# nk4517/gaussian-splatting-skysphere

Hardware: AMD Instinct MI355X
Metric: train iters/sec (fwd+bwd) + render Mpix/s @1080p, 1M Gaussians SH=3 (higher is better)
Workload: dtype f32; 1 GPU; C3: 1M Gaussians SH3 1920x1080, 16x16 tiles; gaussians=1000000, sh_degree=3, width=1920, height=1080, render_exp2=hardware v_exp_f32, parallelism=view-parallel dp1

## Files before the change

### gaussian-splatting-skysphere_amd/csrc/gs_api.hip

```cpp
#include <dlfcn.h>

#include <atomic>
#include <cstdlib>
#include <stdarg.h>
#include <stdio.h>
#include <string.h>

#include <mutex>
#include <string>
#include <vector>

#include "../../include/gsrast.h"
#include "gs_internal.h"

namespace gs {

static thread_local std::string t_err;
static thread_local bool t_failed = false;
static thread_local bool t_debug = false;

static void set_error(const char* fmt, ...) {
  if (t_failed) return;
  char buf[1024];
  va_list ap;
// ... 202 lines not shown
  }
  if (rgb) {
    rgb[3 * i] = b.z;
    rgb[3 * i + 1] = b.w;
    rgb[3 * i + 2] = d.x;
  }
  if (depth) depth[i] = d.y;
}

}

using namespace gs;

namespace gs {
static std::atomic<int> g_exact_exp{-1};
bool exact_exp() {
  int v = g_exact_exp.load(std::memory_order_relaxed);
  if (v < 0) {
    const char* e = getenv("GSRAST_EXACT_EXP");
    v = (e && e[0] && e[0] != '0') ? 1 : 0;
    g_exact_exp.store(v, std::memory_order_relaxed);
  }
  return v != 0;
}
}

namespace gs {
static std::atomic<uint32_t> g_spin_limit{LB_SPIN_LIMIT};
uint32_t scan_spin_limit() { return g_spin_limit.load(std::memory_order_relaxed); }
static std::atomic<int> g_tile_sort_packed{1};
static std::atomic<long long> g_tile_sort_packed_n{0};
bool tile_sort_packed() { return g_tile_sort_packed.load(std::memory_order_relaxed) != 0; }
void tile_sort_packed_note() { g_tile_sort_packed_n.fetch_add(1, std::memory_order_relaxed); }

static thread_local RowWait t_row_waits[GS_MAX_ROW_WAITS];
static thread_local int t_row_wait_count = 0;
int take_row_waits(RowWait* out, int max) {
  const int n = t_row_wait_count < max ? t_row_wait_count : max;
  for (int k = 0; k < n; k++) out[k] = t_row_waits[k];
  t_row_wait_count = 0;
  return n;
}
bool stream_wait(hipStream_t st, hipEvent_t ev) {
  const hipError_t e = hipStreamWaitEvent(st, ev, 0);
  if (e != hipSuccess) set_error("row wait: hipStreamWaitEvent failed: %s", hipGetErrorString(e));
  return e == hipSuccess;
}
uint32_t next_scan_epoch() {
  static std::atomic<uint32_t> e{0};
  return (e.fetch_add(1, std::memory_order_relaxed) % ((1u << 30) - 1u)) + 1u;
}
}

extern "C" {

int gs_abi_version(void) { return GSRAST_ABI_VERSION; }
const char* gs_last_error(void) { return t_err.c_str(); }

size_t gs_geom_buffer_bytes(int P) { return geom_layout((size_t)(P > 0 ? P : 1), nullptr, nullptr); }
size_t gs_binning_buffer_bytes(long long num_rendered, int W, int H) {
  if (size_query_refused(W, H)) return 0;
  int tiles = ((W + GS_TILE - 1) / GS_TILE) * ((H + GS_TILE - 1) / GS_TILE);
  return bin_layout((size_t)(num_rendered > 0 ? num_rendered : 1), tiles, nullptr, nullptr);
}
size_t gs_image_buffer_bytes(int W, int H) {
  if (size_query_refused(W, H)) return 0;
// ... 1213 lines not shown
  bwd_gaussians_adam(g, c, geo, a, (hipStream_t)stream);
  return t_failed ? 1 : 0;
}

int gs_mark_visible(int P, const float* means3D, const float* viewmatrix, const float* projmatrix, uint8_t* present,
                    void* stream) {
  clear_error(0);
  if (P < 0) return set_error("P must be >= 0"), 1;
  if (P > 0 && (!means3D || !viewmatrix || !present)) return set_error("missing pointer"), 1;
  mark_visible(P, means3D, viewmatrix, projmatrix, present, (hipStream_t)stream);
  return t_failed ? 1 : 0;
}

size_t gs_knn_scratch_bytes(int P) { return knn_scratch_bytes(P); }

int gs_knn_mean_dist2(int P, const float* points, float* out, void* scratch, void* stream) {
  clear_error(0);
  if (P < 0) return set_error("P must be >= 0"), 1;
  if (P == 0) return 0;
  if (!points || !out || !scratch) return set_error("missing pointer"), 1;
  knn_mean_dist2(P, points, out, (char*)scratch, (hipStream_t)stream);
  return t_failed ? 1 : 0;
}

unsigned gs_debug_set_scan_spin_limit(unsigned limit) {
  return gs::g_spin_limit.exchange(limit, std::memory_order_relaxed);
}

int gs_debug_set_tile_sort_packed(int on) {
  return gs::g_tile_sort_packed.exchange(on ? 1 : 0, std::memory_order_relaxed);
}
long long gs_debug_tile_sort_packed_count(void) { return gs::g_tile_sort_packed_n.load(std::memory_order_relaxed); }

int gs_debug_sh_rows_staged(int D, int M, const void* shs) { return gs::sh_rows_stageable(D, M, shs) ? 1 : 0; }

int gs_debug_launch_log(int enable) {
  const int prev = gs::launch_log_on();
  gs::g_launch_log.store(enable ? 1 : 0, std::memory_order_relaxed);
  return prev;
}

long long gs_debug_launched_kernels(char* buf, long long cap) {
  std::string out;
  {
    std::lock_guard<std::mutex> lk(gs::g_launch_mu);
    for (const void* k : gs::g_launched) {
      Dl_info info;
      if (dladdr(k, &info) && info.dli_sname && info.dli_saddr == k)
        out += info.dli_sname;
      else
        out += "?";
      out += '\n';
    }
  }
  if (buf && cap > (long long)out.size()) memcpy(buf, out.c_str(), out.size() + 1);
  return (long long)out.size();
}

int gs_set_exact_exp(int exact) {
  const int prev = exact_exp() ? 1 : 0;
  gs::g_exact_exp.store(exact ? 1 : 0, std::memory_order_relaxed);
  return prev;
}

size_t gs_ssim_partial_count(int planes, int H, int W) { return ssim_partial_count(planes, H, W); }

// ... 364 lines not shown
```

### gaussian-splatting-skysphere_amd/csrc/gs_backward.hip

```cpp
#include "gs_internal.h"

namespace gs {

#ifdef GS_TIMING
GS_TIMING_BUFFER(g_bwd_timing, gs_debug_bwd_timing)
#define GS_BWD_T0() const unsigned long long t_start = timing_stamp()
#define GS_BWD_TREC(tile, n_eff, walked, slots) timing_record(g_bwd_timing, t_start, tile, n_eff, walked, slots)
#else
#define GS_BWD_T0() (void)0
#define GS_BWD_TREC(tile, n_eff, walked, slots) (void)0
#endif

struct __attribute__((aligned(4))) Rec3 {
  float a, b, c;
};

__device__ __forceinline__ void load_rec(const float* p, float* v) {
  const Rec3* r = reinterpret_cast<const Rec3*>(p);
  const Rec3 a = r[0], b = r[1], c = r[2];
  v[0] = a.a, v[1] = a.b, v[2] = a.c, v[3] = b.a, v[4] = b.b, v[5] = b.c, v[6] = c.a, v[7] = c.b, v[8] = c.c;
}


struct BwdSlot {
// ... 18 lines not shown
  if constexpr (EXACT) inv = __builtin_fmaf(inv, __builtin_fmaf(-omA, inv, 1.0f), inv);
  const float Tn = q.T * inv;
  const float dch = ae * Tn;
  float Cd = __builtin_fmaf(bl, q.d2, __builtin_fmaf(xr.w, q.d1, xr.z * q.d0));
  if constexpr (AUX) Cd = __builtin_fmaf(br.w, q.gD, Cd);
  const float dLa = __builtin_fmaf(Tn, Cd, -(q.U * inv));
  const float qq = oGm * dLa;
  const float mx = dx - br.y, my = dy - br.z;
  const float qx = qq * mx, qy = qq * my;
  s[0] = __builtin_fmaf(dch, q.d0, s[0]);
  s[1] = __builtin_fmaf(dch, q.d1, s[1]);
  s[2] = __builtin_fmaf(dch, q.d2, s[2]);
  s[3] = s[3] + qx;
  s[4] = s[4] + qy;
  s[5] = __builtin_fmaf(qx, mx, s[5]);
  s[6] = __builtin_fmaf(qx, my, s[6]);
  s[7] = __builtin_fmaf(qy, my, s[7]);
  s[8] = s[8] + qq;
  if constexpr (AUX) s[9] = __builtin_fmaf(dch, q.gD, s[9]);
  if constexpr (ABS) {
    constexpr int A0 = AUX ? GRAD_REC + 1 : GRAD_REC;
    const float hx = __builtin_fmaf(co.x + co.x, dx, co.y * dy);
    const float hy = __builtin_fmaf(co.z + co.z, dy, co.y * dx);
    s[A0] = __builtin_fmaf(__builtin_fabsf(qq), __builtin_fabsf(hx), s[A0]);
    s[A0 + 1] = __builtin_fmaf(__builtin_fabsf(qq), __builtin_fabsf(hy), s[A0 + 1]);
  }
  q.T = Tn;
  q.U = __builtin_fmaf(Cd, dch, q.U);
  uint64_t m = __builtin_amdgcn_ballot_w64(c_walk) & __builtin_amdgcn_ballot_w64(c_alpha);
  if constexpr (EXACT) m &= __builtin_amdgcn_ballot_w64(c_pw);
  return m;
}

template <bool EXACT, bool AUX = false, bool ABS = false, class... Abs>
__global__ __launch_bounds__(64) void k_render_bwd_tw(CameraArgs c, const uint2* __restrict__ ranges,
                                                                    const uint32_t* __restrict__ point_list,
                                                                    const uint32_t* __restrict__ point_gid,
                                                                    const float4* __restrict__ splat,
                                                                    const float* __restrict__ final_T,
                                                                    const uint32_t* __restrict__ n_contrib,
                                                                    const uint32_t* __restrict__ tile_max,
                                                                    const uint32_t* __restrict__ tile_order,
                                                                    const float* __restrict__ dL_dpix,
                                                                    float* __restrict__ gradrec, BwdAux aux,
                                                                    Abs... abs) {
  static_assert(sizeof...(Abs) == (ABS ? 1 : 0), "ABS: one BwdAbs argument");
  __shared__ float4 s_xy[64];
  __shared__ float4 s_co[64];
  __shared__ float4 s_br[64];
  constexpr int AOFF = AUX ? 24 : 16;
  constexpr int ROW = ABS ? (AUX ? 36 : 24) : AOFF;
  constexpr int NS = GRAD_REC + (AUX ? 1 : 0) + (ABS ? 2 : 0);
  __shared__ __attribute__((aligned(16))) float s_acc[64][ROW];
  GS_BWD_T0();
  const uint32_t tile = __builtin_amdgcn_readfirstlane(tile_order ? tile_order[blockIdx.x] : blockIdx.x);
  if (tile == ~0u) return;
  const int tx = (int)(tile % (uint32_t)c.gx), ty = (int)(tile / (uint32_t)c.gx);
  const int lane = threadIdx.x;
  const uint2 range = ranges[tile];
  const uint32_t n = range.y - range.x;
  const uint4 qm = reinterpret_cast<const uint4*>(tile_max)[tile];
  const uint32_t qlast[4] = {min(qm.x, n), min(qm.y, n), min(qm.z, n), min(qm.w, n)};
  const uint32_t n_eff = max(max(qlast[0], qlast[1]), max(qlast[2], qlast[3]));
  if (n_eff == 0) {
    GS_BWD_TREC(tile, 0u, 0u, 0u);
    return;
  }
#ifdef GS_TIMING
  uint32_t t_walked = 0, t_slots = 0;
#endif

  const size_t HW = (size_t)c.W * c.H;
  const int qx0 = tx * GS_TILE + (lane & 7), qy0 = ty * GS_TILE + (lane >> 3);
  BwdSlot p[4];
#pragma unroll
  for (int k = 0; k < 4; k++) {
    const int px = qx0 + 8 * (k & 1), py = qy0 + 8 * (k >> 1);
    const bool in = px < c.W && py < c.H;
    const size_t pix = in ? (size_t)py * c.W + px : 0;
    const float Tf = in ? final_T[pix] : 0.0f;
    p[k].T = Tf;
    p[k].last = in ? n_contrib[pix] : 0u;
    p[k].d0 = in ? dL_dpix[pix] : 0.0f;
    p[k].d1 = in ? dL_dpix[HW + pix] : 0.0f;
    p[k].d2 = in ? dL_dpix[2 * HW + pix] : 0.0f;
    p[k].U = Tf * (c.bg[0] * p[k].d0 + c.bg[1] * p[k].d1 + c.bg[2] * p[k].d2);
    if constexpr (AUX) {
      const float gA = in && aux.d_alpha ? aux.d_alpha[pix] : 0.0f;
      p[k].U = p[k].U - Tf * gA;
      p[k].gD = in && aux.d_invdepth ? aux.d_invdepth[pix] : 0.0f;
    }
  }
  const float ddelx_dx = (float)(0.5 * c.W), ddely_dy = (float)(0.5 * c.H);
  const float pfx0 = (float)qx0, pfy0 = (float)qy0;
  using lds_float = __attribute__((address_space(3))) float;
  lds_float* const acc_lane = (lds_float*)(&s_acc[0][(lane >> 4) + 4 * ((lane >> 3) & 1)]);
  const bool hi8 = (lane & 8) != 0;

  const int32_t e0 = (int32_t)n_eff - 1 - lane;
  const uint32_t* const plist = point_list + range.x;
  auto pos = [&](int32_t e) { return (uint32_t)max(e, 0); };
  uint32_t slot_c = plist[pos(e0)];
  uint32_t G1 = point_gid[slot_c];
  float4 pa = splat[3 * G1], pb = splat[3 * G1 + 1], pd = splat[3 * G1 + 2];
  uint32_t S1 = plist[pos(e0 - 64)];
  G1 = point_gid[S1];
  uint32_t S2 = plist[pos(e0 - 128)];

  uint32_t rec_lanes = 0;
  auto store_records = [&]() {
    if ((uint32_t)lane < rec_lanes) {
      const float4* row = reinterpret_cast<const float4*>(&s_acc[lane][0]);
      const float4 a = row[0], b = row[1], d = row[2];
      Rec3* r = reinterpret_cast<Rec3*>(gradrec + (size_t)__float_as_uint(d.y) * GRAD_REC);
      r[0] = Rec3{a.x, a.y, a.z};
      r[1] = Rec3{a.w, b.x, b.y};
      r[2] = Rec3{b.z, b.w, d.x};
      if constexpr (AUX) aux.gradrec_aux[__float_as_uint(d.y)] = d.z;
      if constexpr (ABS) {
        const float4 ea = row[3];
        reinterpret_cast<float2*>((abs, ...).gradrec_abs)[__float_as_uint(d.y)] = make_float2(ea.x, ea.y);
      }
    }
  };
  for (uint32_t base = 0; base < n_eff; base += 64) {
    const uint32_t cnt = min(64u, n_eff - base);
    const bool mine = (uint32_t)lane < cnt;
    const uint32_t slot = slot_c;
    const float ccx = pa.z, ccy = pa.w, ccz = pb.x, cop = pb.y;
    uint32_t qmask = 0;
    if (mine) {
      s_xy[lane] = make_float4(pa.x, pa.y, pb.z, pb.w);
      s_co[lane] = fall_coefs_m<EXACT>(pa.z, pa.w, pb.x, pb.y);
      const float x0 = (float)(tx * GS_TILE), y0 = (float)(ty * GS_TILE);
      s_br[lane] = make_float4(pd.x, pa.x - fminf(fmaxf(pa.x, x0), x0 + 15.0f),
// ... 79 lines not shown
        if constexpr (ABS) {
          const float4 b0 = *reinterpret_cast<const float4*>(&s_acc[lane][AOFF]);
          const float4 b1 = *reinterpret_cast<const float4*>(&s_acc[lane][AOFF + 4]);
          S[NS - 2] = (b0.x + b1.x) + (b0.y + b1.y);
          S[NS - 1] = (b0.z + b1.z) + (b0.w + b1.w);
        }
      } else {
#pragma unroll
        for (int t = 0; t < NS; t++) S[t] = 0.0f;
      }
      const float2 R = *reinterpret_cast<const float2*>(&s_br[lane].y);
      const double Rx = R.x, Ry = R.y, q0 = S[8];
      const float m1x = (float)__builtin_fma(Rx, q0, (double)S[3]), m1y = (float)__builtin_fma(Ry, q0, (double)S[4]);
      __builtin_amdgcn_sched_barrier(0);
      const float m2xx = (float)__builtin_fma(Rx, __builtin_fma(Rx, q0, 2.0 * (double)S[3]), (double)S[5]);
      __builtin_amdgcn_sched_barrier(0);
      const float m2xy = (float)__builtin_fma(Rx, __builtin_fma(Ry, q0, (double)S[4]),
                                              __builtin_fma(Ry, (double)S[3], (double)S[6]));
      __builtin_amdgcn_sched_barrier(0);
      const float m2yy = (float)__builtin_fma(Ry, __builtin_fma(Ry, q0, 2.0 * (double)S[4]), (double)S[7]);
      __builtin_amdgcn_sched_barrier(0);
      float4* row = reinterpret_cast<float4*>(&s_acc[lane][0]);
      row[0] = make_float4(S[0], S[1], S[2], -ddelx_dx * (ccx * m1x + ccy * m1y));
      row[1] = make_float4(-ddely_dy * (ccz * m1y + ccy * m1x), -0.5f * m2xx, -0.5f * m2xy, -0.5f * m2yy);
      float s9 = 0.0f;
      if constexpr (AUX) s9 = S[9];
      row[2] = make_float4(S[8] != 0.0f ? S[8] / cop : 0.0f, __uint_as_float(slot), s9, 0.0f);
      if constexpr (ABS) row[3] = make_float4(S[NS - 2], S[NS - 1], 0.0f, 0.0f);
    }
    rec_lanes = cnt;
    __builtin_amdgcn_wave_barrier();
  }
  store_records();
  GS_BWD_TREC(tile, n_eff, t_walked, t_slots);
}

constexpr int ORDER_THREADS = 256;
__global__ __launch_bounds__(ORDER_THREADS) void k_tile_order(const uint32_t* __restrict__ len_hist,
                                                              const uint32_t* __restrict__ tile_brank, uint32_t gx,
                                                              uint32_t gy, uint32_t* __restrict__ order,
                                                              const uint32_t* __restrict__ tile_max,
                                                              const uint2* __restrict__ ranges,
                                                              const uint32_t* __restrict__ point_list,
                                                              uint32_t* __restrict__ tile_cut,
                                                              uint32_t* __restrict__ cut_max) {
  __shared__ uint32_t s_base[ORDER_GROUPS][ORDER_BUCKETS];
  const uint32_t tid = threadIdx.x, t = blockIdx.x * ORDER_THREADS + tid, lane = tid & 63, wid = tid >> 6;
  const uint32_t tiles = gx * gy;
  uint32_t cut = 0;
  if (t < tiles) {
    const uint4 q = reinterpret_cast<const uint4*>(tile_max)[t];
    const uint2 r = ranges[t];
    const uint32_t n_eff = min(max(max(q.x, q.y), max(q.z, q.w)), r.y - r.x);
    cut = n_eff ? point_list[r.x + n_eff - 1] + 1u : 0u;
    tile_cut[t] = cut;
  }
  {
    const uint32_t wm = wave_max_u32(cut);
    if (lane == 0 && wm) atomicMax(cut_max, wm);
  }
  if (!order) return;
  const uint32_t br = t < tiles ? tile_brank[t] : 0u;
  static_assert(ORDER_BUCKETS == 64 && ORDER_GROUPS == 2 * (ORDER_THREADS / 64), "two groups per wave");
#pragma unroll
  for (int h = 0; h < 2; h++) {
    const uint32_t g = wid + h * (ORDER_THREADS / 64);
    const uint32_t v = len_hist[g * ORDER_BUCKETS + lane];
    s_base[g][lane] = wave_incl_scan(v) - v;
  }
  lds_barrier();
  if (t < tiles) {
    const uint32_t g = t % ORDER_GROUPS;
    order[ORDER_GROUPS * (s_base[g][br >> 22] + (br & 0x3FFFFFu)) + g] = t;
  }
}

void bwd_tile_order(const CameraArgs& c, const BinPtrs& bin, const ImgPtrs& img, hipStream_t st) {
  const uint32_t slots = (uint32_t)(c.gx * c.gy);
  GS_LAUNCH("tile_order", k_tile_order, dim3((slots + ORDER_THREADS - 1) / ORDER_THREADS), dim3(ORDER_THREADS), 0, st,
            img.len_hist, img.tile_brank, (uint32_t)c.gx, (uint32_t)c.gy, img.tile_order, img.tile_max, img.ranges,
            bin.point_list, img.tile_cut, img.cut_max);
}

void bwd_render(int P, const CameraArgs& c, const GeomPtrs& geo, const BinPtrs& bin, const ImgPtrs& img,
                const float* dL_dpix, float* gradrec, hipStream_t st, const BwdAux& aux, const BwdAbs& ab) {
  const int tiles = c.gx * c.gy;
  uint32_t* order = img.tile_order;
  const uint32_t slots = (uint32_t)tiles;
  bwd_tile_order(c, bin, img, st);
  auto launch = [&](const char* name, const char* name_aux, auto... abs) {
    with_flag(aux.on(), [&](auto AUX) {
      with_flag(exact_exp(), [&](auto EXACT) {
        constexpr bool E = decltype(EXACT)::value, A = decltype(AUX)::value;
        GS_LAUNCH(A ? name_aux : name, (k_render_bwd_tw<E, A, sizeof...(abs) != 0, decltype(abs)...>), dim3(slots),
                  dim3(64), 0, st, c, img.ranges, bin.point_list, bin.presort_gid, geo.splat, img.final_T,
                  img.n_contrib, img.tile_max, order, dL_dpix, gradrec, aux, abs...);
      });
    });
  };
  if (ab.on())
    launch("render_bwd_abs", "render_bwd_aux_abs", ab);
  else
    launch("render_bwd", "render_bwd_aux");
}

constexpr int SUMREC_WAVES = 4;
template <int CTRL, int ROW_MASK, int NC = GRAD_REC>
__device__ __forceinline__ void seg_scan_step(float* v, uint32_t own1) {
  const uint32_t o = (uint32_t)__builtin_amdgcn_update_dpp(0, (int)own1, CTRL, ROW_MASK, 0xF, false);
  const float f = o == own1 ? 1.0f : 0.0f;
#pragma unroll
  for (int c = 0; c < NC; c++) v[c] = __builtin_fmaf(dpp_f<CTRL, ROW_MASK>(v[c]), f, v[c]);
}

template <bool AUX = false, bool ABS = false, class... Abs>
__global__ __launch_bounds__(64 * SUMREC_WAVES) void k_sum_records(const uint32_t* __restrict__ counters,
                                                                   const uint32_t* __restrict__ offsets,
                                                                   const uint32_t* __restrict__ sorted_gid,
                                                                   const uint32_t* __restrict__ slot_tile,
                                                                   const uint32_t* __restrict__ tile_cut,
                                                                   const uint32_t* __restrict__ cut_max,
                                                                   const float* __restrict__ gradrec,
                                                                   float* __restrict__ gsum, uint32_t P,
                                                                   const float* __restrict__ gradrec_aux,
                                                                   float* __restrict__ gsum_aux, Abs... abs) {
  static_assert(sizeof...(Abs) == (ABS ? 1 : 0), "ABS: one BwdAbs argument");
  constexpr int A0 = AUX ? GRAD_REC + 1 : GRAD_REC;
  constexpr int NC = A0 + (ABS ? 2 : 0);
  [[maybe_unused]] const float2* gradrec_abs = nullptr;
// ... 1270 lines not shown
```

### gaussian-splatting-skysphere_amd/csrc/gs_forward.hip

```cpp
#include "gs_internal.h"

namespace gs {


template <int DEG>
__device__ __forceinline__ void sh_row_load(const float* __restrict__ sh, const float* __restrict__ rest, bool split,
                                            int M, float* s) {
  constexpr int K = (DEG + 1) * (DEG + 1);
  if (split) {
    const F3 d = *reinterpret_cast<const F3*>(sh);
    s[0] = d.a, s[1] = d.b, s[2] = d.c;
    const F3* r3 = reinterpret_cast<const F3*>(rest);
#pragma unroll
    for (int j = 0; j < K - 1; j++) {
      const F3 t = r3[j];
      s[3 + 3 * j] = t.a, s[4 + 3 * j] = t.b, s[5 + 3 * j] = t.c;
    }
  } else if (((M * 3) & 3) == 0) {
    const float4* s4 = reinterpret_cast<const float4*>(sh);
#pragma unroll
    for (int v = 0; v < (K * 3 + 3) / 4; v++) {
      float4 q = s4[v];
      if (4 * v + 0 < K * 3) s[4 * v + 0] = q.x;
      if (4 * v + 1 < K * 3) s[4 * v + 1] = q.y;
// ... 921 lines not shown
        m_cu &= ~m_stop;
        const bool cu = __builtin_amdgcn_inverse_ballot_w64(m_cu);
        px.C0 = cu ? px.C0 + rr * al[u] * px.T : px.C0;
        px.C1 = cu ? px.C1 + rg * al[u] * px.T : px.C1;
        px.C2 = cu ? px.C2 + rb * al[u] * px.T : px.C2;
        if constexpr (AUX) px.D = cu ? px.D + rd * al[u] * px.T : px.D;
        px.T = cu ? tT : px.T;
        px.last = cu ? __float_as_uint(bl.y) : px.last;
      } else {
        const float tT = __builtin_fmaf(-al[u], px.T, px.T);
        const uint64_t m_keep = __builtin_amdgcn_ballot_w64(tT >= 0.0001f);
        px.done |= m_cu & ~m_keep;
        m_cu &= m_keep;
        const bool cu = __builtin_amdgcn_inverse_ballot_w64(m_cu);
        const float wgt = cu ? al[u] * px.T : 0.0f;
        px.C0 = __builtin_fmaf(rr, wgt, px.C0);
        px.C1 = __builtin_fmaf(rg, wgt, px.C1);
        px.C2 = __builtin_fmaf(rb, wgt, px.C2);
        if constexpr (AUX) px.D = __builtin_fmaf(rd, wgt, px.D);
        px.T = cu ? tT : px.T;
        px.last = cu ? __float_as_uint(bl.y) : px.last;
      }
    }
    if (px.done == ~0ull) break;
  }
}

#ifdef GS_TIMING
GS_TIMING_BUFFER(g_fwd_timing, gs_debug_fwd_timing)
#endif

__device__ __forceinline__ void tile_finish(uint32_t tile, uint32_t grp, uint32_t wave_last,
                                            uint64_t* __restrict__ tile_done, uint32_t* __restrict__ len_hist,
                                            uint32_t* __restrict__ tile_brank) {
  const uint32_t cls = min((uint32_t)(4.0f * __log2f((float)wave_last + 1.0f)), 47u);
  const uint64_t mine = (1ull << (8 + cls)) + 1ull;
  const uint64_t old = atomicAdd((unsigned long long*)&tile_done[tile], (unsigned long long)mine);
  if ((old & 7ull) != 3ull) return;
  const uint32_t top = 63u - (uint32_t)__builtin_clzll((old + mine) >> 8);
  const uint32_t b = (uint32_t)ORDER_BUCKETS - 1u - top;
  tile_brank[tile] = b << 22 | atomicAdd(&len_hist[grp * ORDER_BUCKETS + b], 1u);
}

__device__ __forceinline__ void fwd_store(const CameraArgs& c, const QuadPix& q, bool inside, const FwdPix& px,
                                          float* __restrict__ out, float* __restrict__ final_T,
                                          uint32_t* __restrict__ n_contrib) {
  if (inside) {
    const size_t pix = (size_t)q.py * c.W + q.px, HW = (size_t)c.W * c.H;
    final_T[pix] = px.T;
    n_contrib[pix] = px.last;
    out[pix] = px.C0 + px.T * c.bg[0];
    out[HW + pix] = px.C1 + px.T * c.bg[1];
    out[2 * HW + pix] = px.C2 + px.T * c.bg[2];
  }
}
__device__ __forceinline__ void fwd_store_aux(const CameraArgs& c, const QuadPix& q, bool inside, const FwdPix& px,
                                              float* __restrict__ out_invdepth, float* __restrict__ out_alpha) {
  if (inside) {
    const size_t pix = (size_t)q.py * c.W + q.px;
    if (out_invdepth) out_invdepth[pix] = px.D;
    if (out_alpha) out_alpha[pix] = 1.0f - px.T;
  }
}

constexpr int FWDQ_NB = 64;
constexpr int FWDQ_NBS = FWDQ_NB + 1;
template <bool EXACT, bool AUX = false>
__global__ __launch_bounds__(64) void k_render_fwd_q(CameraArgs c, const uint2* __restrict__ ranges,
                                                     const uint32_t* __restrict__ point_list,
                                                     const uint32_t* __restrict__ point_gid,
                                                     const float4* __restrict__ splat, float* __restrict__ out,
                                                     ImgPtrs img, const uint32_t* __restrict__ err,
                                                     uint32_t* __restrict__ err_host, FwdAux aux) {
  __shared__ float4 s_ent[3 * FWDQ_NBS];
// ... 21 lines not shown
  FwdPix px;
  px.done = __builtin_amdgcn_ballot_w64(!inside);
  for (uint32_t base = 0; base < n; base += FWDQ_NB) {
    if (px.done == ~0ull) break;
    bool meets = false;
    if (lane < (uint32_t)FWDQ_NB && base + lane < n) {
      const uint32_t gid = point_gid[point_list[range.x + base + lane]];
      const float4 a = splat[3 * gid], bb = splat[3 * gid + 1], d = splat[3 * gid + 2];
      s_ent[lane] = make_float4(a.x, a.y, bb.z, bb.w);
      s_ent[FWDQ_NBS + lane] = fall_coefs_m<EXACT>(a.z, a.w, bb.x, bb.y);
      s_ent[2 * FWDQ_NBS + lane] =
          make_float4(d.x, __uint_as_float(base + lane + 1), AUX ? 1.0f / d.y : 0.0f, 0.0f);
      meets = d.z >= 0.0f && ellipse_meets_rect(a.x, a.y, a.z, a.w, bb.x, d.z, qx, qx + 7.0f, qy, qy + 7.0f);
    }
    const uint64_t m = __ballot(meets);
    if (meets)
      s_qlist[__builtin_amdgcn_mbcnt_hi((uint32_t)(m >> 32), __builtin_amdgcn_mbcnt_lo((uint32_t)m, 0u))] =
          16u * lane;
    const uint32_t qcnt = (uint32_t)__popcll(m);
    if (lane < 2 * FWD_ILP) s_qlist[qcnt + lane] = 16u * FWDQ_NB;
    __builtin_amdgcn_wave_barrier();
#ifdef GS_TIMING
    t_batches++;
    t_walked += qcnt;
#endif
    fwd_walk<EXACT, FWDQ_NBS, AUX>(ent, s_qlist, qcnt, (float)q.px, (float)q.py, px);
    __builtin_amdgcn_wave_barrier();
  }
  fwd_store(c, q, inside, px, out, img.final_T, img.n_contrib);
  if constexpr (AUX) fwd_store_aux(c, q, inside, px, aux.invdepth, aux.alpha);
  const uint32_t wmax = wave_max_u32(px.last);
  if (lane == 0) {
    img.tile_max[4 * tile + wid] = wmax;
    tile_finish(tile, tile % ORDER_GROUPS, wmax, img.tile_done, img.len_hist, img.tile_brank);
  }
#ifdef GS_TIMING
  timing_record(g_fwd_timing, t_start, tile, (uint32_t)wid | n << 2, t_batches, t_walked);
#endif
}

void fwd_render(const CameraArgs& c, const GeomPtrs& geo, const BinPtrs& bin, const ImgPtrs& img, float* out_color,
                hipStream_t st, uint32_t* err_host, const FwdAux& aux) {
  const int tiles = c.gx * c.gy;
  const int blocks = (int)xcd_span((uint32_t)tiles) * 32;
  with_flag(aux.invdepth || aux.alpha, [&](auto AUX) {
    with_flag(exact_exp(), [&](auto EXACT) {
      GS_LAUNCH(decltype(AUX)::value ? "render_fwd_aux" : "render_fwd",
                (k_render_fwd_q<decltype(EXACT)::value, decltype(AUX)::value>), dim3(blocks), dim3(64), 0, st, c,
                img.ranges, bin.point_list, bin.presort_gid, geo.splat, out_color, img, &geo.counters[CNT_ERR], err_host,
                aux);
    });
  });
}

__global__ __launch_bounds__(256) void k_mark_visible(int P, const float* __restrict__ means,
                                                      const float* __restrict__ view, uint8_t* __restrict__ present) {
  const int i = blockIdx.x * 256 + threadIdx.x;
  if (i >= P) return;
  const float3v pv = xf43(view, means[3 * i], means[3 * i + 1], means[3 * i + 2]);
  present[i] = !(pv.z <= 0.2f);
}

void mark_visible(int P, const float* means3D, const float* view, const float* proj, uint8_t* present,
                  hipStream_t st) {
  (void)proj;
  if (P <= 0) return;
  GS_LAUNCH("mark_visible", k_mark_visible, dim3((P + 255) / 256), dim3(256), 0, st, P, means3D, view, present);
// ... 4 lines not shown
```

### gaussian-splatting-skysphere_amd/csrc/gs_internal.h

```cpp
#pragma once
#include <stddef.h>
#include <stdint.h>

#include <cmath>
#include <type_traits>

#include "../../include/gsrast.h"
#include "gs_common.h"
#include "gs_sortscan.h"

namespace gs {

bool exact_exp();


constexpr int GRAD_REC = 9;

inline size_t align_up(size_t x) { return (x + 255) & ~(size_t)255; }

constexpr uint32_t DUP_SLOTS = 2048;
__host__ __device__ inline bool dup_balanced(uint32_t I, uint32_t P) {
  return (uint64_t)I <= (uint64_t)DUP_SLOTS * (uint64_t)P;
}

// ... 178 lines not shown
    out->vals_a = (uint32_t*)(base + o_va);
    out->keys_b = (uint32_t*)(base + o_kb);
    out->vals_b = (uint32_t*)(base + o_vb);
    out->offsets = (uint32_t*)(base + o_offs);
    out->rtiles_a = (uint32_t*)(base + o_rta);
    out->rtiles_b = (uint32_t*)(base + o_rtb);
    out->tiles_by_rank = (radix_passes(32) % 2 == 0) ? out->rtiles_b : out->rtiles_a;
    out->dup_first = (uint32_t*)(base + o_df);
    out->gsum = (float*)(base + o_gs);
    out->scan_partial = (uint32_t*)(base + o_sp);
    out->lb_status = (uint64_t*)(base + o_lb);
    out->sort_scratch = (uint32_t*)(base + o_ss);
    out->counters = (uint32_t*)(base + o_cnt);
    out->wg_tot = (WgTotals*)(base + o_wg);
    out->sorted_gid = (radix_passes(32) % 2 == 0) ? out->vals_a : out->vals_b;
  }
  return off;
}

struct BinPtrs {
  uint32_t *keys_a, *vals_a, *keys_b, *vals_b;
  uint32_t* presort_gid;
  uint32_t* sort_scratch;
  uint32_t* point_list;
  uint32_t* sorted_tile;
  uint32_t* slot_tile;
  uint32_t* count;
  uint32_t* pack_tab;
};

constexpr size_t PACK_SCRATCH_WORDS = (size_t)RADIX * RADIX;
bool tile_sort_packed();
void tile_sort_packed_note();



inline int tile_bits(int tiles) {
  int b = 1;
  while (b < 32 && ((uint64_t)1 << b) < (uint64_t)tiles) b++;
  return b;
}

inline size_t bin_layout(size_t I, int tiles, BinPtrs* out, char* base) {
  size_t off = 0;
  auto take = [&](size_t bytes) {
    size_t o = off;
    off += align_up(bytes);
    return o;
  };
  size_t In = I ? I : 1;
  size_t o_ka = take(In * 4), o_va = take(In * 4), o_kb = take(In * 4), o_vb = take(In * 4);
  size_t o_pg = take(In * 4), o_st = take(In * 4);
  size_t o_ss = take((sort_scratch_words(In) + PACK_SCRATCH_WORDS) * 4);
  size_t o_cn = take(64);
  size_t o_pt = take(PACK_TAB_WORDS * 4);
  if (out && base) {
    out->count = (uint32_t*)(base + o_cn);
    out->pack_tab = (uint32_t*)(base + o_pt);
    out->keys_a = (uint32_t*)(base + o_ka);
    out->vals_a = (uint32_t*)(base + o_va);
    out->keys_b = (uint32_t*)(base + o_kb);
    out->vals_b = (uint32_t*)(base + o_vb);
    out->presort_gid = (uint32_t*)(base + o_pg);
    out->slot_tile = (uint32_t*)(base + o_st);
    out->sort_scratch = (uint32_t*)(base + o_ss);
    bool in_b = radix_passes(tile_bits(tiles)) % 2 == 1;
    out->point_list = in_b ? out->vals_b : out->vals_a;
    out->sorted_tile = in_b ? out->keys_b : out->keys_a;
  }
  return off;
}

struct ImgPtrs {
  uint2* ranges;
  float* final_T;
  uint32_t* n_contrib;
  uint32_t* tile_max;
  uint32_t* tile_order;
  uint32_t* tile_cut;
  uint64_t* tile_done;
  uint32_t* len_hist;
  uint32_t* tile_brank;
  uint32_t* cut_max;
};

constexpr int ORDER_BUCKETS = 64;
inline uint32_t sched_words(uint32_t tiles);

constexpr int ORDER_GROUPS = 8;
inline uint32_t sched_words(uint32_t tiles) { return 2u * tiles + ORDER_GROUPS * ORDER_BUCKETS + 1u; }
__host__ __device__ inline uint32_t xcd_span(uint32_t tiles) { return (tiles + ORDER_GROUPS - 1) / ORDER_GROUPS; }
__host__ __device__ inline uint32_t xcd_tile(uint32_t g, uint32_t k, uint32_t gx, uint32_t gy) {
  const uint32_t t = ORDER_GROUPS * k + g;
  return t < gx * gy ? t : ~0u;
}

inline size_t img_layout(int W, int H, ImgPtrs* out, char* base) {
  size_t off = 0;
  auto take = [&](size_t bytes) {
    size_t o = off;
    off += align_up(bytes);
    return o;
  };
  size_t tiles = (size_t)((W + GS_TILE - 1) / GS_TILE) * ((H + GS_TILE - 1) / GS_TILE);
  size_t npix = (size_t)W * H;
  if (tiles == 0) tiles = 1;
  if (npix == 0) npix = 1;
  size_t o_r = take(tiles * 8), o_t = take(npix * 4), o_n = take(npix * 4), o_m = take(tiles * 16),
         o_o = take(tiles * 4), o_c = take(tiles * 4), o_d = take((size_t)sched_words((uint32_t)tiles) * 4),
         o_b = take(tiles * 4);
  if (out && base) {
    out->ranges = (uint2*)(base + o_r);
    out->final_T = (float*)(base + o_t);
    out->n_contrib = (uint32_t*)(base + o_n);
    out->tile_max = (uint32_t*)(base + o_m);
    out->tile_order = (uint32_t*)(base + o_o);
    out->tile_cut = (uint32_t*)(base + o_c);
    out->tile_done = (uint64_t*)(base + o_d);
    out->len_hist = (uint32_t*)(out->tile_done + tiles);
    out->cut_max = out->len_hist + ORDER_GROUPS * ORDER_BUCKETS;
    out->tile_brank = (uint32_t*)(base + o_b);
  }
  return off;
}

#ifdef GS_TIMING
constexpr int TIMING_MAX = 1 << 16;
#define GS_TIMING_BUFFER(buf, fn)                                                                   \
  __device__ unsigned long long buf[TIMING_MAX][5];                                                 \
  extern "C" int fn(unsigned long long* host_out, int n, int reset) {                               \
    if (n > TIMING_MAX) n = TIMING_MAX;                                                             \
    if (host_out && hipMemcpyFromSymbol(host_out, HIP_SYMBOL(buf), (size_t)n * 5 * 8) != hipSuccess) \
      return 1;                                                                                     \
    if (reset) {                                                                                    \
      void* p = nullptr;                                                                            \
      if (hipGetSymbolAddress(&p, HIP_SYMBOL(buf)) != hipSuccess) return 1;                          \
      if (hipMemset(p, 0, sizeof(buf)) != hipSuccess || hipDeviceSynchronize() != hipSuccess) return 1; \
    }                                                                                               \
    return 0;                                                                                       \
  }
__device__ __forceinline__ unsigned long long timing_stamp() {
  __builtin_amdgcn_sched_barrier(0);
  const unsigned long long t = __builtin_amdgcn_s_memrealtime();
  __builtin_amdgcn_s_waitcnt(0xC07F);
  __builtin_amdgcn_sched_barrier(0);
  return t;
}
__device__ __forceinline__ void timing_record(unsigned long long (*buf)[5], unsigned long long t0, uint32_t a,
                                              uint32_t b, uint32_t c, uint32_t d) {
  const unsigned long long t1 = timing_stamp();
  if (threadIdx.x == 0 && blockIdx.x < TIMING_MAX) {
    const uint32_t xcc = __builtin_amdgcn_s_getreg((31 << 11) | 20);
    const uint32_t hw = __builtin_amdgcn_s_getreg((31 << 11) | 4);
    unsigned long long* o = buf[blockIdx.x];
// ... 267 lines not shown
```

### gaussian-splatting-skysphere_amd/diff_gaussian_rasterization/_native.py

```python
from __future__ import annotations

import ctypes
import os

_PKG_ROOT = os.path.dirname(os.path.dirname(os.path.abspath(__file__)))
LIB_PATH = os.environ.get("GSRAST_LIB", os.path.join(_PKG_ROOT, "build", "libgsrast.so"))

_c_p = ctypes.c_void_p
_c_i = ctypes.c_int
_c_d = ctypes.c_double
_c_f = ctypes.c_float
_c_ll = ctypes.c_longlong
_c_sz = ctypes.c_size_t



class ViewGrad(ctypes.Structure):
    _fields_ = [("viewmatrix", ctypes.c_void_p), ("projmatrix", ctypes.c_void_p), ("campos", ctypes.c_void_p),
                ("tan_fovx", ctypes.c_float), ("tan_fovy", ctypes.c_float), ("image_width", ctypes.c_int),
                ("image_height", ctypes.c_int), ("geom_buffer", ctypes.c_void_p)]


SIGNATURES = {
    "gs_abi_version": (_c_i, []),
# ... 173 lines not shown
    "gs_sky_camera_scratch_bytes": (_c_sz, [_c_i, _c_i]),
    "gs_sky_compose_backward_camera": (_c_i, [_c_i, _c_i, _c_p, _c_f, _c_f, _c_i, _c_i, _c_p, _c_p, _c_p, _c_p, _c_p,
                                              _c_i, _c_p, _c_p, _c_i, _c_p, _c_p]),
    "gs_mark_visible": (_c_i, [_c_i, _c_p, _c_p, _c_p, _c_p, _c_p]),
    "gs_knn_scratch_bytes": (_c_sz, [_c_i]),
    "gs_knn_mean_dist2": (_c_i, [_c_i, _c_p, _c_p, _c_p, _c_p]),
    "gs_set_exact_exp": (_c_i, [_c_i]),
    "gs_debug_launch_log": (_c_i, [_c_i]),
    "gs_debug_launched_kernels": (_c_ll, [ctypes.c_char_p, _c_ll]),
    "gs_ssim_partial_count": (_c_sz, [_c_i, _c_i, _c_i]),
    "gs_ssim_forward": (_c_i, [_c_i, _c_i, _c_i, _c_p, _c_p, _c_p, _c_p, _c_p, _c_p, _c_p]),
    "gs_ssim_backward": (_c_i, [_c_i, _c_i, _c_i, _c_i, _c_p, _c_p, _c_p, _c_p, _c_p, _c_p, _c_p]),
    "gs_photometric_loss_forward": (_c_i, [_c_i, _c_i, _c_i, _c_p, _c_p, _c_p, _c_f, _c_p, _c_p, _c_p, _c_p]),
    "gs_photometric_loss_backward": (_c_i, [_c_i, _c_i, _c_i, _c_p, _c_p, _c_p, _c_p, _c_f, _c_p, _c_p, _c_p]),
    "gs_adam_step": (_c_i, [_c_i, _c_p, _c_p, _c_p, _c_p, _c_p, _c_p, _c_p, _c_p, _c_d, _c_d, _c_d, _c_i, _c_p]),
    "gs_adam_step_activated": (_c_i, [_c_i, _c_p, _c_p, _c_p, _c_i, _c_p, _c_p, _c_p, _c_p, _c_p, _c_p, _c_d, _c_d, _c_d,
                                      _c_i, _c_p]),
    "gs_activate_forward": (_c_i, [_c_i, _c_i] + [_c_p] * 9 + [_c_p]),
    "gs_activate_backward": (_c_i, [_c_i, _c_i] + [_c_p] * 12 + [_c_p]),
    "gs_densify_block_count": (_c_sz, [_c_i]),
    "gs_densify_classify": (_c_i, [_c_i, _c_p, _c_p, _c_p, _c_p, _c_d, _c_d, _c_d, _c_d, _c_i, _c_d, _c_i, _c_p, _c_p,
                                   _c_p, _c_p]),
    "gs_densify_split_stds": (_c_i, [_c_i, _c_i, _c_p, _c_p, _c_p, _c_p, _c_p, _c_p]),
    "gs_densify_emit": (_c_i, [_c_i, _c_i] + [_c_p] * 12),
    "gs_densify_stats": (_c_i, [_c_i, _c_p, _c_p, _c_i, _c_p, _c_p, _c_p, _c_p]),
    "gs_debug_export": (
        _c_i,
        [_c_i, _c_i, _c_i, _c_ll, _c_p, _c_p, _c_p, _c_p, _c_p, _c_p, _c_p, _c_p, _c_p, _c_p, _c_p, _c_p, _c_p],
    ),
    "gs_debug_export_slots": (_c_i, [_c_i, _c_i, _c_ll, _c_p, _c_p, _c_p, _c_p, _c_p]),
    "gs_debug_set_scan_spin_limit": (ctypes.c_uint, [ctypes.c_uint]),
    "gs_debug_set_tile_sort_packed": (_c_i, [_c_i]),
    "gs_debug_tile_sort_packed_count": (_c_ll, []),
    "gs_debug_sh_rows_staged": (_c_i, [_c_i, _c_i, _c_p]),
    "gs_profile_enable": (None, [_c_i]),
    "gs_profile_collect": (_c_i, []),
    "gs_profile_reset": (None, []),
    "gs_profile_stat": (_c_i, [_c_i, ctypes.c_char_p, _c_i, ctypes.POINTER(ctypes.c_double), ctypes.POINTER(_c_ll)]),
}

_lib = None


def load():
    global _lib
    if _lib is not None:
        return _lib
    if not os.path.exists(LIB_PATH):
        raise ImportError(
            f"libgsrast.so not found at {LIB_PATH}; build it with "
            f"`make -C {_PKG_ROOT}` (hipcc --offload-arch=gfx950). There is no CPU fallback."
        )
    lib = ctypes.CDLL(LIB_PATH, mode=ctypes.RTLD_GLOBAL)
    for name, (res, args) in SIGNATURES.items():
        fn = getattr(lib, name)
        fn.restype = res
        fn.argtypes = args
    _lib = lib
    return lib


def last_error() -> str:
    msg = load().gs_last_error()
    return msg.decode() if msg else "unknown error"


# ... 18 lines not shown
```

### include/gsrast.h

```cpp
#ifndef GSRAST_H
#define GSRAST_H

#include <stddef.h>
#include <stdint.h>

#ifdef __cplusplus
extern "C" {
#endif

#define GSRAST_ABI_VERSION 17

#define GSRAST_HAS_AUX 1

#define GSRAST_HAS_SKY 1

#define GSRAST_HAS_SKY_CAMERA 1

#define GSRAST_HAS_CAMERA_GRAD 1

#define GSRAST_HAS_AUX_DEFERRED 1

#define GSRAST_HAS_ANTIALIASING 1

#define GSRAST_HAS_CONTRIB 1
// ... 341 lines not shown
                        const float* opacity_raw, const float* scaling_raw, const float* rotation_raw, float* shs,
                        float* opacity, float* scales, float* rotations, void* stream);
int gs_activate_backward(int P, int sh_rest, const float* dL_dshs, const float* dL_dopacity, const float* dL_dscales,
                         const float* dL_drotations, const float* opacity, const float* scales,
                         const float* rotation_raw, float* dL_dfeatures_dc, float* dL_dfeatures_rest,
                         float* dL_dopacity_raw, float* dL_dscaling_raw, float* dL_drotation_raw, void* stream);

size_t gs_densify_block_count(int P);
int gs_densify_classify(int P, const float* grad_accum, const float* denom, const float* opacity_raw,
                        const float* scaling_raw, double grad_threshold, double pd_extent, double min_opacity,
                        double big_extent, int has_screen, double max_screen, int N, uint8_t* flags,
                        uint32_t* block_counts, uint32_t* totals, void* stream);
int gs_densify_split_stds(int P, int N, const uint32_t* totals_host, const uint8_t* flags,
                          const uint32_t* block_counts, const float* scaling_raw, float* stds, void* stream);
int gs_densify_emit(int P, int N, const uint32_t* totals_host, const uint8_t* flags, const uint32_t* block_counts,
                    const float* samples, const float* const* params_host, const float* const* exp_avg_host,
                    const float* const* exp_avg_sq_host, float* const* out_params_host,
                    float* const* out_exp_avg_host, float* const* out_exp_avg_sq_host, const int* widths_host,
                    void* stream);

int gs_densify_stats(int P, const int* radii, const float* grad2d, int grad_stride, float* max_radii2D,
                     float* grad_accum, float* denom, void* stream);

int gs_debug_export(int P, int image_width, int image_height, long long num_rendered, const void* geom_buffer,
                    const void* binning_buffer, const void* image_buffer, uint32_t* point_list,
                    uint32_t* ranges, float* xy, float* conic_opacity, float* rgb, float* depth,
                    uint32_t* tiles_touched, float* final_T, uint32_t* n_contrib, void* stream);

unsigned gs_debug_set_scan_spin_limit(unsigned limit);

int gs_debug_set_tile_sort_packed(int on);
long long gs_debug_tile_sort_packed_count(void);

int gs_debug_sh_rows_staged(int D, int M, const void* shs);

int gs_debug_export_slots(int image_width, int image_height, long long num_rendered, const void* binning_buffer,
                          const void* image_buffer, uint32_t* slots, uint32_t* tile_cut, void* stream);

void gs_profile_enable(int on);
int gs_profile_collect(void);
void gs_profile_reset(void);
int gs_profile_stat(int i, char* name, int name_len, double* total_ms, long long* launches);

#ifdef __cplusplus
}
#endif
#endif
```

Baseline: 1308 iters/s.

## Fold backward tile ordering into the render-backward kernel via forward-built bucket members

The forward tile_finish now also writes each tile into a per-group, per-bucket members list. With the new default bwd_fold flag, the backward kernel skips the separate bwd_tile_order pass. Each block instead derives its tile from a wave-level inclusive scan of the length histogram plus a members lookup, and writes tile_cut and cut_max itself. This removes one kernel launch and its memory traffic, at the cost of extra scratch memory, a per-block scan, and atomics in the backward kernel.

```diff
diff --git a/gaussian-splatting-skysphere_amd/csrc/gs_api.hip b/gaussian-splatting-skysphere_amd/csrc/gs_api.hip
--- a/gaussian-splatting-skysphere_amd/csrc/gs_api.hip
+++ b/gaussian-splatting-skysphere_amd/csrc/gs_api.hip
@@ -258,6 +258,8 @@
 static std::atomic<long long> g_tile_sort_packed_n{0};
 bool tile_sort_packed() { return g_tile_sort_packed.load(std::memory_order_relaxed) != 0; }
 void tile_sort_packed_note() { g_tile_sort_packed_n.fetch_add(1, std::memory_order_relaxed); }
+static std::atomic<int> g_bwd_fold{1};
+bool bwd_fold() { return g_bwd_fold.load(std::memory_order_relaxed) != 0; }
 
 static thread_local RowWait t_row_waits[GS_MAX_ROW_WAITS];
 static thread_local int t_row_wait_count = 0;
@@ -1537,6 +1539,8 @@
 }
 long long gs_debug_tile_sort_packed_count(void) { return gs::g_tile_sort_packed_n.load(std::memory_order_relaxed); }
 
+int gs_debug_set_bwd_fold(int on) { return gs::g_bwd_fold.exchange(on ? 1 : 0, std::memory_order_relaxed); }
+
 int gs_debug_sh_rows_staged(int D, int M, const void* shs) { return gs::sh_rows_stageable(D, M, shs) ? 1 : 0; }
 
 int gs_debug_launch_log(int enable) {
diff --git a/gaussian-splatting-skysphere_amd/csrc/gs_backward.hip b/gaussian-splatting-skysphere_amd/csrc/gs_backward.hip
--- a/gaussian-splatting-skysphere_amd/csrc/gs_backward.hip
+++ b/gaussian-splatting-skysphere_amd/csrc/gs_backward.hip
@@ -74,6 +74,13 @@
   return m;
 }
 
+struct BwdFold {
+  const uint32_t* len_hist;
+  const uint32_t* members;
+  uint32_t* tile_cut;
+  uint32_t* cut_max;
+};
+
 template <bool EXACT, bool AUX = false, bool ABS = false, class... Abs>
 __global__ __launch_bounds__(64) void k_render_bwd_tw(CameraArgs c, const uint2* __restrict__ ranges,
                                                                     const uint32_t* __restrict__ point_list,
@@ -85,7 +92,7 @@
                                                                     const uint32_t* __restrict__ tile_order,
                                                                     const float* __restrict__ dL_dpix,
                                                                     float* __restrict__ gradrec, BwdAux aux,
-                                                                    Abs... abs) {
+                                                                    BwdFold fold, Abs... abs) {
   static_assert(sizeof...(Abs) == (ABS ? 1 : 0), "ABS: one BwdAbs argument");
   __shared__ float4 s_xy[64];
   __shared__ float4 s_co[64];
@@ -95,16 +102,33 @@
   constexpr int NS = GRAD_REC + (AUX ? 1 : 0) + (ABS ? 2 : 0);
   __shared__ __attribute__((aligned(16))) float s_acc[64][ROW];
   GS_BWD_T0();
-  const uint32_t tile = __builtin_amdgcn_readfirstlane(tile_order ? tile_order[blockIdx.x] : blockIdx.x);
+  const int lane = threadIdx.x;
+  uint32_t tile;
+  if (tile_order) {
+    tile = __builtin_amdgcn_readfirstlane(tile_order[blockIdx.x]);
+  } else {
+    const uint32_t g = blockIdx.x % ORDER_GROUPS, j = blockIdx.x / ORDER_GROUPS;
+    static_assert(ORDER_BUCKETS == 64, "one bucket per lane");
+    const uint32_t cnt = fold.len_hist[g * ORDER_BUCKETS + lane];
+    const uint32_t incl = wave_incl_scan(cnt);
+    const uint64_t past = __builtin_amdgcn_ballot_w64(j < incl);
+    if (past == 0) return;
+    const int b = __builtin_ctzll(past);
+    const uint32_t rank = j - (uint32_t)__builtin_amdgcn_readlane((int)(incl - cnt), b);
+    tile = __builtin_amdgcn_readfirstlane(
+        fold.members[(size_t)(g * ORDER_BUCKETS + (uint32_t)b) * xcd_span((uint32_t)(c.gx * c.gy)) + rank]);
+    if (tile >= (uint32_t)(c.gx * c.gy)) return;
+  }
   if (tile == ~0u) return;
   const int tx = (int)(tile % (uint32_t)c.gx), ty = (int)(tile / (uint32_t)c.gx);
-  const int lane = threadIdx.x;
   const uint2 range = ranges[tile];
   const uint32_t n = range.y - range.x;
+  const uint32_t cut_seen = tile_order ? ~0u : *fold.cut_max;
   const uint4 qm = reinterpret_cast<const uint4*>(tile_max)[tile];
   const uint32_t qlast[4] = {min(qm.x, n), min(qm.y, n), min(qm.z, n), min(qm.w, n)};
   const uint32_t n_eff = max(max(qlast[0], qlast[1]), max(qlast[2], qlast[3]));
   if (n_eff == 0) {
+    if (!tile_order && lane == 0) fold.tile_cut[tile] = 0u;
     GS_BWD_TREC(tile, 0u, 0u, 0u);
     return;
   }
@@ -112,6 +136,10 @@
   uint32_t t_walked = 0, t_slots = 0;
 #endif
 
+  const int32_t e0 = (int32_t)n_eff - 1 - lane;
+  const uint32_t* const plist = point_list + range.x;
+  auto pos = [&](int32_t e) { return (uint32_t)max(e, 0); };
+  uint32_t slot_c = plist[pos(e0)];
   const size_t HW = (size_t)c.W * c.H;
   const int qx0 = tx * GS_TILE + (lane & 7), qy0 = ty * GS_TILE + (lane >> 3);
   BwdSlot p[4];
@@ -133,16 +161,14 @@
       p[k].gD = in && aux.d_invdepth ? aux.d_invdepth[pix] : 0.0f;
     }
   }
+  const uint32_t cut = (uint32_t)__builtin_amdgcn_readfirstlane((int)slot_c) + 1u;
+  if (!tile_order && lane == 0) fold.tile_cut[tile] = cut;
   const float ddelx_dx = (float)(0.5 * c.W), ddely_dy = (float)(0.5 * c.H);
   const float pfx0 = (float)qx0, pfy0 = (float)qy0;
   using lds_float = __attribute__((address_space(3))) float;
   lds_float* const acc_lane = (lds_float*)(&s_acc[0][(lane >> 4) + 4 * ((lane >> 3) & 1)]);
   const bool hi8 = (lane & 8) != 0;
 
-  const int32_t e0 = (int32_t)n_eff - 1 - lane;
-  const uint32_t* const plist = point_list + range.x;
-  auto pos = [&](int32_t e) { return (uint32_t)max(e, 0); };
-  uint32_t slot_c = plist[pos(e0)];
   uint32_t G1 = point_gid[slot_c];
   float4 pa = splat[3 * G1], pb = splat[3 * G1 + 1], pd = splat[3 * G1 + 2];
   uint32_t S1 = plist[pos(e0 - 64)];
@@ -288,6 +314,7 @@
     __builtin_amdgcn_wave_barrier();
   }
   store_records();
+  if (!tile_order && lane == 0 && cut > cut_seen) atomicMax(fold.cut_max, cut);
   GS_BWD_TREC(tile, n_eff, t_walked, t_slots);
 }
 
@@ -341,16 +368,20 @@
 void bwd_render(int P, const CameraArgs& c, const GeomPtrs& geo, const BinPtrs& bin, const ImgPtrs& img,
                 const float* dL_dpix, float* gradrec, hipStream_t st, const BwdAux& aux, const BwdAbs& ab) {
   const int tiles = c.gx * c.gy;
-  uint32_t* order = img.tile_order;
   const uint32_t slots = (uint32_t)tiles;
-  bwd_tile_order(c, bin, img, st);
+  const uint32_t* order = nullptr;
+  if (!bwd_fold()) {
+    bwd_tile_order(c, bin, img, st);
+    order = img.tile_order;
+  }
+  const BwdFold fold{img.len_hist, img.members, img.tile_cut, img.cut_max};
   auto launch = [&](const char* name, const char* name_aux, auto... abs) {
     with_flag(aux.on(), [&](auto AUX) {
       with_flag(exact_exp(), [&](auto EXACT) {
         constexpr bool E = decltype(EXACT)::value, A = decltype(AUX)::value;
         GS_LAUNCH(A ? name_aux : name, (k_render_bwd_tw<E, A, sizeof...(abs) != 0, decltype(abs)...>), dim3(slots),
                   dim3(64), 0, st, c, img.ranges, bin.point_list, bin.presort_gid, geo.splat, img.final_T,
-                  img.n_contrib, img.tile_max, order, dL_dpix, gradrec, aux, abs...);
+                  img.n_contrib, img.tile_max, order, dL_dpix, gradrec, aux, fold, abs...);
       });
     });
   };
diff --git a/gaussian-splatting-skysphere_amd/csrc/gs_forward.hip b/gaussian-splatting-skysphere_amd/csrc/gs_forward.hip
--- a/gaussian-splatting-skysphere_amd/csrc/gs_forward.hip
+++ b/gaussian-splatting-skysphere_amd/csrc/gs_forward.hip
@@ -977,14 +977,17 @@
 
 __device__ __forceinline__ void tile_finish(uint32_t tile, uint32_t grp, uint32_t wave_last,
                                             uint64_t* __restrict__ tile_done, uint32_t* __restrict__ len_hist,
-                                            uint32_t* __restrict__ tile_brank) {
+                                            uint32_t* __restrict__ tile_brank, uint32_t* __restrict__ members,
+                                            uint32_t span) {
   const uint32_t cls = min((uint32_t)(4.0f * __log2f((float)wave_last + 1.0f)), 47u);
   const uint64_t mine = (1ull << (8 + cls)) + 1ull;
   const uint64_t old = atomicAdd((unsigned long long*)&tile_done[tile], (unsigned long long)mine);
   if ((old & 7ull) != 3ull) return;
   const uint32_t top = 63u - (uint32_t)__builtin_clzll((old + mine) >> 8);
   const uint32_t b = (uint32_t)ORDER_BUCKETS - 1u - top;
-  tile_brank[tile] = b << 22 | atomicAdd(&len_hist[grp * ORDER_BUCKETS + b], 1u);
+  const uint32_t rank = atomicAdd(&len_hist[grp * ORDER_BUCKETS + b], 1u);
+  tile_brank[tile] = b << 22 | rank;
+  if (rank < span) members[(size_t)(grp * ORDER_BUCKETS + b) * span + rank] = tile;
 }
 
 __device__ __forceinline__ void fwd_store(const CameraArgs& c, const QuadPix& q, bool inside, const FwdPix& px,
@@ -1072,7 +1075,8 @@
   const uint32_t wmax = wave_max_u32(px.last);
   if (lane == 0) {
     img.tile_max[4 * tile + wid] = wmax;
-    tile_finish(tile, tile % ORDER_GROUPS, wmax, img.tile_done, img.len_hist, img.tile_brank);
+    tile_finish(tile, tile % ORDER_GROUPS, wmax, img.tile_done, img.len_hist, img.tile_brank, img.members,
+                xcd_span((uint32_t)(c.gx * c.gy)));
   }
 #ifdef GS_TIMING
   timing_record(g_fwd_timing, t_start, tile, (uint32_t)wid | n << 2, t_batches, t_walked);
diff --git a/gaussian-splatting-skysphere_amd/csrc/gs_internal.h b/gaussian-splatting-skysphere_amd/csrc/gs_internal.h
--- a/gaussian-splatting-skysphere_amd/csrc/gs_internal.h
+++ b/gaussian-splatting-skysphere_amd/csrc/gs_internal.h
@@ -234,6 +234,7 @@
 constexpr size_t PACK_SCRATCH_WORDS = (size_t)RADIX * RADIX;
 bool tile_sort_packed();
 void tile_sort_packed_note();
+bool bwd_fold();
 
 
 
@@ -284,6 +285,7 @@
   uint32_t* len_hist;
   uint32_t* tile_brank;
   uint32_t* cut_max;
+  uint32_t* members;
 };
 
 constexpr int ORDER_BUCKETS = 64;
@@ -311,6 +313,7 @@
   size_t o_r = take(tiles * 8), o_t = take(npix * 4), o_n = take(npix * 4), o_m = take(tiles * 16),
          o_o = take(tiles * 4), o_c = take(tiles * 4), o_d = take((size_t)sched_words((uint32_t)tiles) * 4),
          o_b = take(tiles * 4);
+  size_t o_mb = take((size_t)ORDER_GROUPS * ORDER_BUCKETS * xcd_span((uint32_t)tiles) * 4);
   if (out && base) {
     out->ranges = (uint2*)(base + o_r);
     out->final_T = (float*)(base + o_t);
@@ -322,6 +325,7 @@
     out->len_hist = (uint32_t*)(out->tile_done + tiles);
     out->cut_max = out->len_hist + ORDER_GROUPS * ORDER_BUCKETS;
     out->tile_brank = (uint32_t*)(base + o_b);
+    out->members = (uint32_t*)(base + o_mb);
   }
   return off;
 }
diff --git a/gaussian-splatting-skysphere_amd/diff_gaussian_rasterization/_native.py b/gaussian-splatting-skysphere_amd/diff_gaussian_rasterization/_native.py
--- a/gaussian-splatting-skysphere_amd/diff_gaussian_rasterization/_native.py
+++ b/gaussian-splatting-skysphere_amd/diff_gaussian_rasterization/_native.py
@@ -229,6 +229,7 @@
     "gs_debug_set_scan_spin_limit": (ctypes.c_uint, [ctypes.c_uint]),
     "gs_debug_set_tile_sort_packed": (_c_i, [_c_i]),
     "gs_debug_tile_sort_packed_count": (_c_ll, []),
+    "gs_debug_set_bwd_fold": (_c_i, [_c_i]),
     "gs_debug_sh_rows_staged": (_c_i, [_c_i, _c_i, _c_p]),
     "gs_profile_enable": (None, [_c_i]),
     "gs_profile_collect": (_c_i, []),
diff --git a/include/gsrast.h b/include/gsrast.h
--- a/include/gsrast.h
+++ b/include/gsrast.h
@@ -397,6 +397,8 @@
 int gs_debug_set_tile_sort_packed(int on);
 long long gs_debug_tile_sort_packed_count(void);
 
+int gs_debug_set_bwd_fold(int on);
+
 int gs_debug_sh_rows_staged(int D, int M, const void* shs);
 
 int gs_debug_export_slots(int image_width, int image_height, long long num_rendered, const void* binning_buffer,
```

Measured after the change: 1311 iters/s, median of 5. No clear change (+0.2%).
